# ZhangT-tech/MoCA-Video

Hardware: AMD Instinct MI355X
Metric: denoising UNet-steps/sec @16x320x512 fp16 (higher is better)
Workload: dtype f16

## Files before the change

include/moca_hip.h:

```cpp
#ifndef MOCA_HIP_H
#define MOCA_HIP_H

#include <stdint.h>

#ifdef __cplusplus
extern "C" {
#endif

#define MOCA_OK            0
#define MOCA_E_BADARG     -1
#define MOCA_E_LAUNCH     -2
#define MOCA_E_NODEVICE   -3
#define MOCA_E_GRAPH      -4

#define MOCA_A_LINEAR   0
#define MOCA_A_CONV3X3  1
#define MOCA_A_TCONV3   2

#define MOCA_EP_GEGLU   1
#define MOCA_EP_OUT_F32 2
#define MOCA_FORCE_SMALL_TILE 4
#define MOCA_EP_COLSUM 16
#define MOCA_EP_LN     32
#define MOCA_EP_GELU    8
// ... 60 lines not shown
int moca_gemm_rowsum_cols(const moca_gemm_params* p);
int moca_gemm_lnfold_ok(const moca_gemm_params* p);
int moca_gemm_tattn_ok(const moca_gemm_params* p);
int moca_gemm_wgroup_ok(const moca_gemm_params* p);
int moca_gemm_cat_ok(const moca_gemm_params* p);
#define MOCA_ROUTE_SMALL64   1
#define MOCA_ROUTE_SMALL128  2
#define MOCA_ROUTE_GLDS128   3
#define MOCA_ROUTE_GLDS160   4
#define MOCA_ROUTE_G4        5
#define MOCA_ROUTE_W80       6
#define MOCA_ROUTE_W80W      7
#define MOCA_ROUTE_SQ256     8
#define MOCA_ROUTE_G4P       9
#define MOCA_ROUTE_SQP       10
#define MOCA_ROUTE_TATTN     11
#define MOCA_ROUTE_WS        12
int moca_gemm_route(const moca_gemm_params* p);
int moca_gemm_splitk_groupnorm_ok(const moca_gemm_params* p, int32_t HW, int32_t frames_per_stat);
int moca_gemm_splitk_groupnorm_f16(const moca_gemm_params* p, void* y, const float* gamma, const float* beta, int32_t HW,
                                   int32_t frames_per_stat, float eps, int32_t silu, int32_t write_x, void* stream);
int64_t moca_gemm_splitk_ws_bytes(int32_t M, int32_t N, int32_t splits);

int moca_groupnorm_nhwc_f16(const void* x, void* y, const float* gamma, const float* beta,
                            int32_t F, int32_t HW, int32_t C, int32_t frames_per_stat,
                            float eps, int32_t silu, float* ws, void* stream);
int64_t moca_groupnorm_ws_bytes(int32_t F, int32_t HW, int32_t C);
int moca_groupnorm_colsum_f16(const void* x, void* y, const float* gamma, const float* beta, const float* colsum,
                              int32_t tile_rows, int32_t F, int32_t HW, int32_t C, int32_t frames_per_stat,
                              float eps, int32_t silu, float* ws, void* stream);

int moca_groupnorm_fold_weights_f16(const void* w, const float* bias, const float* gamma, const float* beta, const int64_t* gstat,
                                    void* wg, float* bg, int32_t n_sg, int32_t N, int32_t K, int32_t ldw, int64_t count, float eps,
                                    void* stream);

int moca_groupnorm_gstat_f16(const void* x, void* y, const float* gamma, const float* beta, const int64_t* gstat,
                             int32_t F, int32_t HW, int32_t C, int32_t frames_per_stat,
                             float eps, int32_t silu, void* stream);
int moca_concat_channels_gstat_f16(const void* a, const void* b, void* out, int32_t F, int32_t HW, int32_t C1, int32_t C2,
                                   int32_t frames_per_stat, int64_t* gstat, void* stream);
int moca_groupnorm_gstat_cat_f16(const void* a, const void* b, void* y, const float* gamma, const float* beta,
                                 const int64_t* gstat_cat, const int64_t* gstat_b, int32_t Fb, int32_t F, int32_t HW, int32_t C1,
                                 int32_t C2, int32_t frames_per_stat, float eps, int32_t silu, void* stream);
int moca_gstat_accum_f16(const void* x, int32_t F, int32_t HW, int32_t C, int32_t frames_per_stat, int32_t cpg, int32_t coff,
                         int64_t* gstat, void* stream);
int moca_memset_zero(void* ptr, int64_t bytes, void* stream);
// ... 163 lines not shown
```

moca_video_amd/lib.py:

```python
from __future__ import annotations

import ctypes as C
import os

import torch

_HERE = os.path.dirname(os.path.abspath(__file__))
LIB_PATH = os.environ.get("MOCA_HIP_LIB") or os.path.join(_HERE, "libmoca_hip.so")

MOCA_A_LINEAR, MOCA_A_CONV3X3, MOCA_A_TCONV3 = 0, 1, 2
MOCA_EP_GEGLU, MOCA_EP_OUT_F32, MOCA_FORCE_SMALL_TILE, MOCA_EP_GELU, MOCA_EP_COLSUM, MOCA_EP_LN = 1, 2, 4, 8, 16, 32
MOCA_EP_ROWSUM, MOCA_EP_LNFOLD, MOCA_EP_GSTAT, MOCA_EP_TATTN, MOCA_EP_SLABS = 64, 128, 256, 512, 1024
MOCA_TUNE_GEMM_W80, MOCA_TUNE_GEMM_G4, MOCA_TUNE_GEMM_SQ256, MOCA_TUNE_GEMM_WIDE, MOCA_TUNE_GN_SLAB, MOCA_TUNE_GEMM_G4P, MOCA_TUNE_GEMM_MF32, MOCA_TUNE_GEMM_SQP, MOCA_TUNE_SQP_WALK = 0, 1, 2, 3, 4, 5, 6, 7, 8
MOCA_TUNE_SLAB_F16 = 9
MOCA_TUNE_GEMM_WS = 10
(MOCA_ROUTE_SMALL64, MOCA_ROUTE_SMALL128, MOCA_ROUTE_GLDS128, MOCA_ROUTE_GLDS160, MOCA_ROUTE_G4, MOCA_ROUTE_W80, MOCA_ROUTE_W80W,
 MOCA_ROUTE_SQ256, MOCA_ROUTE_G4P, MOCA_ROUTE_SQP, MOCA_ROUTE_TATTN, MOCA_ROUTE_WS) = range(1, 13)

_ERR = {0: "ok", -1: "bad argument (shape/alignment contract)", -2: "HIP launch/runtime error",
        -3: "no gfx950 device", -4: "graph capture/replay failed"}


class MocaHipError(RuntimeError):
    pass
# ... 30 lines not shown
    _fields_ = [
        ("state", C.c_void_p), ("x", C.c_void_p), ("eps_c", C.c_void_p), ("eps_u", C.c_void_p), ("noise", C.c_void_p),
        ("momentum", C.c_void_p), ("queue", C.c_void_p), ("x_prev", C.c_void_p), ("pred_x0", C.c_void_p), ("coef", C.c_void_p),
        ("win_start", C.c_void_p), ("mask", C.c_void_p), ("mask_sums", C.c_void_p), ("mask_frame", C.c_void_p),
        ("enh", C.c_void_p), ("cond", C.c_void_p), ("sam_eff", C.c_void_p), ("sam_idx", C.c_void_p),
        ("cfg_scale", C.c_float), ("beta", C.c_float), ("one_minus_beta", C.c_float), ("gamma", C.c_float),
        ("one_minus_gamma", C.c_float),
        ("nW", C.c_int32), ("C", C.c_int32), ("Q", C.c_int32), ("f", C.c_int32), ("HW", C.c_int32), ("wb_from", C.c_int32),
    ]


_vp, _i32, _i64, _f32, _f64 = C.c_void_p, C.c_int32, C.c_int64, C.c_float, C.c_double
SIGNATURES = {
    "moca_gemm_f16": (C.c_int, [C.POINTER(GemmParams), _vp]),
    "moca_gemm_splitk_ws_bytes": (_i64, [_i32, _i32, _i32]),
    "moca_gemm_colsum_rows": (C.c_int, [C.POINTER(GemmParams)]),
    "moca_gemm_ln_ok": (C.c_int, [C.POINTER(GemmParams)]),
    "moca_gemm_rowsum_cols": (C.c_int, [C.POINTER(GemmParams)]),
    "moca_gemm_lnfold_ok": (C.c_int, [C.POINTER(GemmParams)]),
    "moca_gemm_tattn_ok": (C.c_int, [C.POINTER(GemmParams)]),
    "moca_gemm_cat_ok": (C.c_int, [C.POINTER(GemmParams)]),
    "moca_gemm_wgroup_ok": (C.c_int, [C.POINTER(GemmParams)]),
    "moca_gemm_route": (C.c_int, [C.POINTER(GemmParams)]),
    "moca_groupnorm_fold_weights_f16": (C.c_int, [_vp, _vp, _vp, _vp, _vp, _vp, _vp, _i32, _i32, _i32, _i32, _i64, _f32, _vp]),
    "moca_gemm_splitk_groupnorm_ok": (C.c_int, [C.POINTER(GemmParams), _i32, _i32]),
    "moca_gemm_splitk_groupnorm_f16": (C.c_int, [C.POINTER(GemmParams), _vp, _vp, _vp, _i32, _i32, _f32, _i32, _i32, _vp]),
    "moca_groupnorm_gstat_cat_f16": (C.c_int, [_vp, _vp, _vp, _vp, _vp, _vp, _vp, _i32, _i32, _i32, _i32, _i32, _i32, _f32, _i32, _vp]),
    "moca_gstat_accum_f16": (C.c_int, [_vp, _i32, _i32, _i32, _i32, _i32, _i32, _vp, _vp]),
    "moca_groupnorm_colsum_f16": (C.c_int, [_vp, _vp, _vp, _vp, _vp, _i32, _i32, _i32, _i32, _i32, _f32, _i32, _vp, _vp]),
    "moca_groupnorm_nhwc_f16": (C.c_int, [_vp, _vp, _vp, _vp, _i32, _i32, _i32, _i32, _f32, _i32, _vp, _vp]),
    "moca_groupnorm_ws_bytes": (_i64, [_i32, _i32, _i32]),
    "moca_groupnorm_gstat_f16": (C.c_int, [_vp, _vp, _vp, _vp, _vp, _i32, _i32, _i32, _i32, _f32, _i32, _vp]),
    "moca_memset_zero": (C.c_int, [_vp, _i64, _vp]),
    "moca_concat_channels_gstat_f16": (C.c_int, [_vp, _vp, _vp, _i32, _i32, _i32, _i32, _i32, _vp, _vp]),
    "moca_layernorm_f16": (C.c_int, [_vp, _vp, _vp, _vp, _i32, _i32, _f32, _vp]),
    "moca_attention_f16": (C.c_int, [_vp, _vp, _vp, _vp, _i32, _i32, _i32, _i32, _i32, _i32, _i32, _i32, _i32, _f32, _vp]),
    "moca_attention_ip_f16": (C.c_int, [_vp, _vp, _vp, _vp, _vp, _vp] + [_i32] * 12 + [_f32, _f32, _vp]),
    "moca_attention_causal_f16": (C.c_int, [_vp, _vp, _vp, _vp, _i32, _i32, _i32, _i32, _i32, _i32, _i32, _f32, _vp]),
    "moca_embed_tokens_f16": (C.c_int, [_vp, _vp, _vp, _vp, _i32, _i32, _i32, _i32, _vp]),
    "moca_attention_d80_f16": (C.c_int, [_vp, _vp, _vp, _vp, _i32, _i32, _i32, _i32, _i32, _i32, _i32, _f32, _vp]),
    "moca_clip_preprocess_patches_f16": (C.c_int, [_vp, _i32, _vp, _i32, _i32, _i32, _i32, _i32, _i32, _i32, _vp]),
    "moca_clip_assemble_tokens_f16": (C.c_int, [_vp, _i32, _vp, _vp, _vp, _i32, _i32, _i32, _vp]),
    "moca_temporal_attention_f16": (C.c_int, [_vp, _vp, _vp, _vp, _i32, _i32, _i32, _i32, _i32, _i32, _f32, _vp]),
    "moca_temporal_attention_causal_f16": (C.c_int, [_vp, _vp, _vp, _vp, _i32, _i32, _i32, _i32, _i32, _i32, _f32, _vp]),
    "moca_ncthw_to_nhwc_f16": (C.c_int, [_vp, _i32, _vp, _i32, _i32, _i32, _i32, _i32, _vp]),
    "moca_ncthw_scatter_f16": (C.c_int, [_vp, _i32, _vp, _i32, _i32, _i32, _i32, _i32, _i32, _vp]),
# ... 101 lines not shown
```

moca_video_amd/ops.py:

```python
from __future__ import annotations

import ctypes as C
import os
import torch

from . import lib as _l

_stream = None


def set_stream(handle):
    global _stream
    _stream = handle


def current_stream():
    if _stream is None:
        return torch.cuda.current_stream().cuda_stream
    return _stream


def _st():
    return C.c_void_p(current_stream())


def _round_up(x, m):
    return (x + m - 1) // m * m


class PackedWeight:
    __slots__ = ("w", "bias", "N", "K", "n_out", "geglu", "wsum", "derived")

    def __init__(self, w, bias, N, K, n_out, geglu=False):
        self.w, self.bias, self.N, self.K, self.n_out, self.geglu = w, bias, N, K, n_out, geglu
        self.wsum = None
        self.derived = False


def _finish(w2d: torch.Tensor, bias, device, n_out=None, geglu=False) -> PackedWeight:
    n, k = w2d.shape
    npad, kpad = _round_up(n, 64), _round_up(k, 64)
    w = torch.zeros(npad, kpad, dtype=torch.float16, device=device)
    w[:n, :k] = w2d.to(device=device, dtype=torch.float16)
    b = None
    if bias is not None:
        b = torch.zeros(npad, dtype=torch.float32, device=device)
        b[:n] = bias.to(device=device, dtype=torch.float32)
    return PackedWeight(w, b, npad, k, n if n_out is None else n_out, geglu)


def pack_linear(weight, bias=None, device="cuda"):
    w = weight.reshape(weight.shape[0], -1)
    return _finish(w, bias, device)


def pack_linear_cat(weights, biases=None, device="cuda"):
    w = torch.cat([x.reshape(x.shape[0], -1) for x in weights], dim=0)
    b = None
    if biases is not None:
# ... 106 lines not shown
    if tattn is not None:
        p.flags |= _l.MOCA_EP_TATTN
        p.T, p.HW, p.tattn_scale = tattn[:3]
        p.tattn_causal = 1 if len(tattn) > 3 and tattn[3] else 0
    if gstat is not None:
        p.flags |= _l.MOCA_EP_GSTAT
        p.gstat = gstat[0].data_ptr()
        p.gstat_rows = gstat[1]
        if len(gstat) > 2:
            p.gstat_cpg, p.gstat_coff = gstat[2], gstat[3]
    if lnfold is not None:
        p.flags |= _l.MOCA_EP_LNFOLD
        p.lnf_part = lnfold[0].data_ptr() if lnfold[0] is not None else None
        p.lnf_nparts = lnfold[1]
        p.ln_eps = lnfold[2]
        p.lnf_wsum = pw.wsum.data_ptr() if pw.wsum is not None else None
    if slabs:
        p.flags |= _l.MOCA_EP_SLABS
    p.splits = splits
    return p


def gemm(a, pw: PackedWeight, out, **kw):
    p = _gemm_params(a, pw, out, **kw)
    _l.check(_l.load().moca_gemm_f16(C.byref(p), _st()), "moca_gemm_f16")
    return out


def gemm_ln_ok(a, pw: PackedWeight, **kw):
    p = _gemm_params(a, pw, None, **kw)
    return bool(_l.load().moca_gemm_ln_ok(C.byref(p)))


def gemm_rowsum_cols(a, pw: PackedWeight, **kw):
    p = _gemm_params(a, pw, None, **kw)
    return int(_l.load().moca_gemm_rowsum_cols(C.byref(p)))


def gemm_lnfold_ok(a, pw: PackedWeight, **kw):
    p = _gemm_params(a, pw, None, **kw)
    return bool(_l.load().moca_gemm_lnfold_ok(C.byref(p)))


def gemm_wgroup_ok(a, pw: PackedWeight, **kw):
    p = _gemm_params(a, pw, None, **kw)
    return bool(_l.load().moca_gemm_wgroup_ok(C.byref(p)))


def gemm_route(a, pw: PackedWeight, out=None, **kw):
    p = _gemm_params(a, pw, out, **kw)
    return int(_l.load().moca_gemm_route(C.byref(p)))


def groupnorm_fold_weights(pw: PackedWeight, gamma, beta, gstat, wg, bg, *, n_sg, count, eps):
    _l.check(_l.load().moca_groupnorm_fold_weights_f16(_l.ptr(pw.w), _l.ptr(pw.bias) if pw.bias is not None else None, _l.ptr(gamma), _l.ptr(beta),
                                                       _l.ptr(gstat), _l.ptr(wg), _l.ptr(bg), n_sg, pw.N, pw.K, pw.w.stride(0), count, eps, _st()),
             "moca_groupnorm_fold_weights_f16")
    out = PackedWeight(wg, bg, pw.N, pw.K, pw.n_out)
    out.derived = True
    return out


def gemm_tattn_ok(a, pw: PackedWeight, **kw):
    p = _gemm_params(a, pw, None, **kw)
    return bool(_l.load().moca_gemm_tattn_ok(C.byref(p)))


def pack_qkv_per_head(wq, wk, wv, heads, bias=None, device="cuda"):
    C_ = wq.shape[0]
    assert C_ == heads * 64 and wk.shape[0] == C_ and wv.shape[0] == C_
    w = torch.stack([wq.reshape(heads, 64, -1), wk.reshape(heads, 64, -1), wv.reshape(heads, 64, -1)], dim=1).reshape(3 * C_, -1)
    b = None
    if bias is not None:
        b = torch.stack([bias[:C_].reshape(heads, 64), bias[C_:2 * C_].reshape(heads, 64), bias[2 * C_:].reshape(heads, 64)], dim=1).reshape(-1)
# ... 211 lines not shown
```

moca_video_amd/plan.py:

```python
from __future__ import annotations

import ctypes as C
import functools
import os
import warnings

import torch

from . import lib as _l
from . import ops
from .unet import (IMAGE_CONTEXT_MAX, TEXT_CONTEXT_LEN, _BasicTransformerBlock, _CatMap, _Downsample, _FMap, _Pool, _ResBlock,
                   _SpatialTransformer, _TemporalTransformer, _Upsample)

N_CU = 256


def gemm_splits(M, pw):
    nk = pw.w.shape[1] // 64
    tiles = 0
    if pw.N % 160 == 0 and not pw.geglu and M > 160:
        tiles = ((M + 319) // 320) * (pw.N // 160)
        if tiles < 200:
            tiles = 0
    if tiles == 0:
        if M > 128 and (pw.N % 128 == 0 or pw.N % 160 == 0):
            tm, bn = 256, (128 if pw.N % 128 == 0 else 160)
        else:
            tm, bn = 128, (128 if pw.N % 128 == 0 else 64)
        tiles = ((M + tm - 1) // tm) * (pw.N // bn)
    if tiles >= (N_CU * 3) // 4:
        return 1
    cap = N_CU // tiles
    if tiles >= 40:
        if nk <= 24:
            return 1
        if nk <= 100:
            return max(1, min(cap, 4))
    return max(1, min(cap, nk // 8))


PREFETCH_MIN_BYTES = int(float(os.environ.get("MOCA_PREFETCH_MIN_MB", "4")) * (1 << 20))
PREFETCH_HOST_FLOP = float(os.environ.get("MOCA_PREFETCH_HOST_GF", "50")) * 1e9
VIRTUAL_CAT = os.environ.get("MOCA_VCAT", "1") != "0"
SPLITK_GN = os.environ.get("MOCA_SKGN", "1") != "0"
GN_FOLD = os.environ.get("MOCA_GNFOLD", "1") != "0"
SPLITK_GN_ALL = os.environ.get("MOCA_SKGN", "1") == "2"


class _LNRef:
    __slots__ = ("x", "part", "nparts")

    def __init__(self, x, part, nparts):
        self.x, self.part, self.nparts = x, part, nparts


class _PlanBase:
    _defer_slabs = False

    def __init__(self, model, device):
        self.model = model
        self.device = device
        self.P = model._packed
        self.pool = _Pool(device)
        self.stream = torch.cuda.Stream(device=device) if torch.device(device).type == "cuda" else None
        self.steps = []
        self._pinned = set()
        self.graph = None
        self.graph_failed = False
# ... 594 lines not shown
        for layer in seq:
            if isinstance(layer, _ResBlock):
                nh = self.res_block(layer, h)
            elif isinstance(layer, _SpatialTransformer):
                nh = self.transformer(layer, h, True)
            elif isinstance(layer, _TemporalTransformer):
                nh = self.transformer(layer, h, False)
            elif isinstance(layer, _Downsample):
                nh = self.conv(h, self.P[id(layer.op)], stride=2)
            elif isinstance(layer, _Upsample):
                nh = self.upconv(h, layer.conv)
            else:
                raise TypeError(type(layer))
            if isinstance(h, _CatMap):
                self._drop_colsum(h.h)
                self._drop_colsum(h.skip)
                self._release(h.h.buf, h.skip.buf)
            else:
                self._release(h.buf)
                self._drop_colsum(h)
            h = nh
        return h

    def _embed_mlp(self, sq, rows_t):
        m, P, BT = self.model, self.P, self.BT
        te = self.pool.get(BT, m.model_channels)
        self._emit(ops.timestep_embedding, rows_t, te, n=BT, dim=m.model_channels)
        e1 = self.linear(te, BT, P[id(sq[0])])
        s1 = self.pool.get(BT, e1.shape[1])
        self._emit(ops.silu_add_rows, e1, 1, None, 1, s1, rows=BT, Cn=e1.shape[1], silu=True)
        e2 = self.linear(s1, BT, P[id(sq[2])])
        self._release(te, e1, s1)
        return e2

    def _build(self):
        m, P, B, T, H, W = self.model, self.P, self.B, self.T, self.H, self.W
        BT = self.BT
        emb = self._embed_mlp(m.time_embed, self.t_rows)
        femb = self._embed_mlp(m.fps_embedding, self.fps_rows) if m.fps_cond else None
        self.emb_silu = self.pool.get(BT, emb.shape[1])
        self._emit(ops.silu_add_rows, emb, 1, femb, 1, self.emb_silu, rows=BT, Cn=emb.shape[1], silu=True)
        self._release(emb, femb)
        self._pinned.add(self.emb_silu.data_ptr())
        self.emb_all = self.linear(self.emb_silu, BT, P["emb_all"])
        self._pinned.add(self.emb_all.data_ptr())
        self.kv_all = None
        if "ctx_kv_all" in P:
            self.kv_all = self.linear(self.ctx, self.ctx_rows, P["ctx_kv_all"])
            self._pinned.add(self.kv_all.data_ptr())
        self.kv_ip_all = None
        if self.ctx_img is not None:
            self.kv_ip_all = self.linear(self.ctx_img, self.img_rows, P["ctx_kv_ip_all"])
            self._pinned.add(self.kv_ip_all.data_ptr())

        FT = self.Bx * T
        Cpad = m.in_cpad
        if self.pieces is None:
            x8 = self.pool.get(FT * H * W, Cpad)
            self._emit(ops.ncthw_to_nhwc, self.x_in, x8, B=self.Bx, Cin=m.in_channels, T=T, HW=H * W, Cpad=Cpad)
            h = self.conv(_FMap(x8, FT, H, W, Cpad), P[id(m.input_blocks[0][0])])
            self._release(x8)
        else:
            self.x_rows = torch.zeros(FT * H * W, Cpad, dtype=torch.float16, device=self.device)
            self._emit(ops.ncthw_scatter, self.x_in, self.x_rows, B=self.Bx, k=self.kx, T=T, HW=H * W, Cpad=Cpad, c0=0)
            h = self.conv(_FMap(self.x_rows, FT, H, W, Cpad), P[id(m.input_blocks[0][0])])
        hs = []
        for i, module in enumerate(m.input_blocks):
            if i == 0:
                if m.addition_attention:
                    nh = self.transformer(m.init_attn[0], h, False)
                    self._release(h.buf)
                    self._drop_colsum(h)
                    h = nh
            else:
                h = self.run_seq(module, h)
            if self.adapter_in is not None and (i + 1) % 3 == 0:
                self._adapter_add(h, FT)
            hs.append(h)
            self._pinned.add(h.buf.data_ptr())
        h = self.run_seq(m.middle_block, h)
        if h.F != BT:
            h = _FMap(self._expand(h.buf, h.M, h.C), BT, h.H, h.W, h.C)
        for module in m.output_blocks:
            skip = hs.pop()
            if skip.F != h.F:
                self._pinned.discard(skip.buf.data_ptr())
                wide = self._expand(skip.buf, skip.M, skip.C)
                self._drop_colsum(skip)
# ... 4 lines not shown
            vc = self._virtual_cat(module, h, skip)
            if vc is not None:
                self._pinned.discard(skip.buf.data_ptr())
                h = self.run_seq(module, vc)
                continue
            cat = self.pool.get(h.M, h.C + skip.C)
            gst = None
            Cc = h.C + skip.C
            if isinstance(module[0], _ResBlock) and Cc % 32 == 0 and \
                    64 <= (Cc // 8) * max(1, 256 // (Cc // 8)) and Cc // 8 <= 1024:
                gst = (self._gstat_slot(h.F * 64), 1)
                self._emit(ops.concat_channels_gstat, h.buf, skip.buf, cat, gst[0], F=h.F, HW=h.H * h.W, C1=h.C, C2=skip.C,
                           frames_per_stat=1)
            else:
                self._emit(ops.concat_channels, h.buf, skip.buf, cat, rows=h.M, C1=h.C, C2=skip.C)
            self._pinned.discard(skip.buf.data_ptr())
            self._drop_colsum(h)
            self._drop_colsum(skip)
            self._release(h.buf, skip.buf)
            h = self.run_seq(module, _FMap(cat, h.F, h.H, h.W, Cc, gstat=gst))
        g = self.gn(h, P[id(m.out[0])], fps=1, eps=1e-5, silu=True)
        self._release(h.buf)
        self._drop_colsum(h)
        o = self.conv(_FMap(g, h.F, h.H, h.W, h.C), P[id(m.out[2])])
        self._release(g)
        self._emit(ops.nhwc_to_ncthw, o.buf, o.C, self.out, B=B, Cout=m.out_channels, T=T, HW=H * W)
        self._release(o.buf)
        self._finish_prefetch()

    def _adapter_add(self, h, FT):
        self._drop_colsum(h)
        assert h.gstat is None and h.gstat_own is None and not h.cs_used
        h.src, h.cs_rows = None, 0
        src = torch.empty(FT, h.C, h.H, h.W, dtype=torch.float32, device=self.device)
        self.adapter_in.append(src)
        self._emit(ops.nchw_add_rows, h.buf, src, F=h.F, Fsrc=FT, Cn=h.C, HW=h.H * h.W)

    def _virtual_cat(self, module, h, skip):
        if not VIRTUAL_CAT or not isinstance(module[0], _ResBlock) or isinstance(module[0].skip_connection, torch.nn.Identity):
            return None
        Cc, HW = h.C + skip.C, h.H * h.W
        if Cc % 32 or h.C % 64 or skip.C % 64 or Cc // 8 > 1024 or h.F != skip.F:
            return None
        pw = self.P[id(module[0].skip_connection)]
        if self._splits(h.M, pw) != 1 or not ops.gemm_cat_ok(h.buf, pw, M=h.M, lda=h.buf.stride(-2), splits=1, a2=(skip.buf, h.C)):
            return None
        gw = Cc // 32
# ... 107 lines not shown
```

Before: 64.85.

## Add specialized kernels for skinny linears, narrow-output and short-K 3x3 convs

```diff
diff --git a/include/moca_hip.h b/include/moca_hip.h
--- a/include/moca_hip.h
+++ b/include/moca_hip.h
@@ -106,6 +106,18 @@
                                    int32_t frames_per_stat, float eps, int32_t silu, int32_t write_x, void* stream);
 int64_t moca_gemm_splitk_ws_bytes(int32_t M, int32_t N, int32_t splits);
 
+int moca_linear_skinny_ok(int32_t M, int32_t N, int32_t K, int32_t lda, int32_t ldw, int32_t ldo);
+int moca_linear_skinny_f16(const void* a, const void* w, const float* bias, void* out, int32_t M, int32_t N, int32_t K,
+                           int32_t lda, int32_t ldw, int32_t ldo, void* stream);
+int moca_conv3x3_narrow_ok(int32_t F, int32_t H, int32_t W, int32_t C, int32_t n_out, int32_t ldw, int32_t ldo);
+int moca_conv3x3_narrow_f16(const void* a, const void* w, const float* bias, void* out, int32_t F, int32_t H, int32_t W,
+                            int32_t C, int32_t n_out, int32_t ldw, int32_t ldo, void* stream);
+int moca_conv3x3_shortk_ok(int32_t F, int32_t H, int32_t W, int32_t Cpad, int32_t N, int32_t ldw, int32_t ldo,
+                           int32_t gstat_rows, int32_t gstat_cpg, int32_t gstat_coff);
+int moca_conv3x3_shortk_f16(const void* a, const void* w, const float* bias, void* out, int64_t* gstat, int32_t F, int32_t H,
+                            int32_t W, int32_t Cpad, int32_t N, int32_t ldw, int32_t ldo, int32_t gstat_rows, int32_t gstat_cpg,
+                            int32_t gstat_coff, void* stream);
+
 int moca_groupnorm_nhwc_f16(const void* x, void* y, const float* gamma, const float* beta,
                             int32_t F, int32_t HW, int32_t C, int32_t frames_per_stat,
                             float eps, int32_t silu, float* ws, void* stream);
diff --git a/moca_video_amd/csrc/small_shapes.hip b/moca_video_amd/csrc/small_shapes.hip
--- /dev/null
+++ b/moca_video_amd/csrc/small_shapes.hip
@@ -0,0 +1,462 @@
+#include "common.h"
+
+namespace {
+
+typedef unsigned u32x4 __attribute__((ext_vector_type(4)));
+[[maybe_unused]] constexpr unsigned SS_OOB = 0x80000000u;
+
+__device__ __forceinline__ __amdgpu_buffer_rsrc_t ss_rsrc(const void* p, int64_t bytes) {
+    return __builtin_amdgcn_make_buffer_rsrc(const_cast<void*>(p), 0, (int)bytes, 0x00020000);
+}
+__device__ __forceinline__ half8v ss_ld16(__amdgpu_buffer_rsrc_t r, unsigned off) {
+    return __builtin_bit_cast(half8v, __builtin_amdgcn_raw_buffer_load_b128(r, (int)off, 0, 0));
+}
+
+int ss_cus() {
+    static int cached = 0;
+    if (!cached) {
+        int dev = 0;
+        hipDeviceProp_t prop;
+        if (hipGetDevice(&dev) == hipSuccess && hipGetDeviceProperties(&prop, dev) == hipSuccess && prop.multiProcessorCount > 0)
+            cached = prop.multiProcessorCount;
+        else
+            cached = 256;
+    }
+    return cached;
+}
+
+template <bool KSPLIT>
+__global__ __launch_bounds__(KSPLIT ? 256 : 512) void skinny_linear_kernel(const half_t* __restrict__ a, const half_t* __restrict__ w,
+                                                                           const float* __restrict__ bias, half_t* __restrict__ out,
+                                                                           int M, int N, int K, int lda, int ldw, int ldo) {
+#if defined(__HIP_DEVICE_COMPILE__)
+    extern __shared__ __attribute__((aligned(16))) char smem[];
+    constexpr int NW = KSPLIT ? 4 : 8, NT = NW * 64;
+    const int tid = threadIdx.x, lane = tid & 63, fr = lane & 15, fq = lane >> 4;
+    const int wave = __builtin_amdgcn_readfirstlane(tid >> 6);
+    const int U = K >> 6, nrb = M > 16 ? 2 : 1;
+    const int ct = KSPLIT ? (int)blockIdx.x : (int)blockIdx.x * NW + wave;
+    const bool live = ct < (N >> 4);
+    int u0 = 0, u1 = U;
+    if constexpr (KSPLIT) {
+        const int upw = (U + NW - 1) / NW;
+        u0 = min(U, wave * upw);
+        u1 = min(U, u0 + upw);
+    }
+    const __amdgpu_buffer_rsrc_t rsrc_w = ss_rsrc(w, (int64_t)N * ldw * 2);
+    const __amdgpu_buffer_rsrc_t rsrc_a = ss_rsrc(a, ((int64_t)(M - 1) * lda + K) * 2);
+    const unsigned wrow = live ? (unsigned)(((ct * 16 + fr) * ldw + 16 * fq) * 2) : SS_OOB;
+    half8v w0[10], w1[10];
+    auto load_w = [&](half8v (&buf)[10], int ub) {
+#pragma unroll
+        for (int i = 0; i < 5; ++i) {
+            const int u = ub + i;
+            const unsigned off = u < u1 ? wrow + (unsigned)u * 128u : SS_OOB;
+            buf[2 * i] = ss_ld16(rsrc_w, off);
+            buf[2 * i + 1] = ss_ld16(rsrc_w, off + 16u);
+        }
+    };
+    load_w(w0, u0);
+
+    const int cpr = K >> 3, total = nrb * 16 * cpr;
+    const int spare = nrb * 16 * K * 2 + (KSPLIT ? NW * 2 * 1024 : 0) + lane * 16;
+    constexpr int AU = 10;
+    for (int base = tid; base < total; base += AU * NT) {
+        half8v v[AU];
+#pragma unroll
+        for (int j = 0; j < AU; ++j) {
+            const int idx = base + j * NT, row = idx / cpr, c = idx - row * cpr;
+            v[j] = ss_ld16(rsrc_a, idx < total && row < M ? (unsigned)((row * lda + c * 8) * 2) : SS_OOB);
+        }
+#pragma unroll
+        for (int j = 0; j < AU; ++j) {
+            const int idx = base + j * NT, row = idx / cpr, c = idx - row * cpr;
+            const int frag = (row >> 4) * 2 * U + 2 * (c >> 3) + (c & 1), l = ((c >> 1) & 3) * 16 + (row & 15);
+            *reinterpret_cast<half8v*>(smem + (idx < total ? (frag * 64 + l) * 16 : spare)) = v[j];
+        }
+    }
+    __syncthreads();
+
+    f32x4 acc0 = {0.f, 0.f, 0.f, 0.f}, acc1 = {0.f, 0.f, 0.f, 0.f};
+    const char* const a_rd = smem + lane * 16;
+    auto compute = [&](const half8v (&buf)[10], int ub) {
+#pragma unroll
+        for (int i = 0; i < 5; ++i) {
+            const int u = ub + i;
+            if (u < u1) {
+#pragma unroll
+                for (int h = 0; h < 2; ++h) {
+                    const half8v a0 = *reinterpret_cast<const half8v*>(a_rd + (2 * u + h) * 1024);
+                    acc0 = __builtin_amdgcn_mfma_f32_16x16x32_f16(buf[2 * i + h], a0, acc0, 0, 0, 0);
+                    if (nrb == 2) {
+                        const half8v a1 = *reinterpret_cast<const half8v*>(a_rd + (2 * U + 2 * u + h) * 1024);
+                        acc1 = __builtin_amdgcn_mfma_f32_16x16x32_f16(buf[2 * i + h], a1, acc1, 0, 0, 0);
+                    }
+                }
+            }
+        }
+    };
+    for (int ub = u0; ub < u1; ub += 10) {
+        load_w(w1, ub + 5);
+        compute(w0, ub);
+        load_w(w0, ub + 10);
+        compute(w1, ub + 5);
+    }
+
+    if constexpr (KSPLIT) {
+        float* const ex = reinterpret_cast<float*>(smem + nrb * 16 * K * 2);
+        *reinterpret_cast<f32x4*>(ex + ((wave * 2 + 0) * 64 + lane) * 4) = acc0;
+        *reinterpret_cast<f32x4*>(ex + ((wave * 2 + 1) * 64 + lane) * 4) = acc1;
+        __syncthreads();
+        if (wave != 0) return;
+        acc0 = *reinterpret_cast<const f32x4*>(ex + lane * 4);
+        acc1 = *reinterpret_cast<const f32x4*>(ex + (64 + lane) * 4);
+#pragma unroll
+        for (int wv = 1; wv < NW; ++wv) {
+            acc0 += *reinterpret_cast<const f32x4*>(ex + ((wv * 2 + 0) * 64 + lane) * 4);
+            acc1 += *reinterpret_cast<const f32x4*>(ex + ((wv * 2 + 1) * 64 + lane) * 4);
+        }
+    }
+    if (!live) return;
+    const int n = ct * 16 + 4 * fq;
+    f32x4 b = {0.f, 0.f, 0.f, 0.f};
+    if (bias) b = *reinterpret_cast<const f32x4*>(bias + n);
+    if (fr < M) {
+        const half4v o = {(half_t)(acc0[0] + b[0]), (half_t)(acc0[1] + b[1]), (half_t)(acc0[2] + b[2]), (half_t)(acc0[3] + b[3])};
+        *reinterpret_cast<half4v*>(out + (int64_t)fr * ldo + n) = o;
+    }
+    if (16 + fr < M) {
+        const half4v o = {(half_t)(acc1[0] + b[0]), (half_t)(acc1[1] + b[1]), (half_t)(acc1[2] + b[2]), (half_t)(acc1[3] + b[3])};
+        *reinterpret_cast<half4v*>(out + (int64_t)(16 + fr) * ldo + n) = o;
+    }
+#endif
+}
+
+[[maybe_unused]] constexpr int NC_G = 5, NC_NL = 9;
+__global__ __launch_bounds__(512) void conv3x3_narrow_kernel(const half_t* __restrict__ a, const half_t* __restrict__ w,
+                                                             const float* __restrict__ bias, half_t* __restrict__ out, int M, int H,
+                                                             int W, int C, int ldw, int ldo) {
+#if defined(__HIP_DEVICE_COMPILE__)
+    extern __shared__ __attribute__((aligned(16))) char smem[];
+    const int tid = threadIdx.x, lane = tid & 63, fr = lane & 15, fq = lane >> 4;
+    const int wave = __builtin_amdgcn_readfirstlane(tid >> 6);
+    const int cs = C >> 5, KS = 9 * cs, ncp = cs >> 1;
+    const int npix = NC_G * 64 + 2 * W + 2;
+    const int zslot = KS * 1024, spare = zslot + 128 + lane * 16, abase = zslot + 128 + 1024;
+    if (tid < 8) *reinterpret_cast<half8v*>(smem + zslot + tid * 16) = half8v{0, 0, 0, 0, 0, 0, 0, 0};
+    const __amdgpu_buffer_rsrc_t rsrc_w = ss_rsrc(w, (int64_t)16 * ldw * 2);
+    for (int base = tid; base < KS * 64; base += 6 * 512) {
+        half8v v[6];
+#pragma unroll
+        for (int j = 0; j < 6; ++j) {
+            const int idx = base + j * 512, sk = idx >> 6, l = idx & 63;
+            v[j] = ss_ld16(rsrc_w, idx < KS * 64 ? (unsigned)(((l & 15) * ldw + 32 * sk + 8 * (l >> 4)) * 2) : SS_OOB);
+        }
+#pragma unroll
+        for (int j = 0; j < 6; ++j) {
+            const int idx = base + j * 512;
+            *reinterpret_cast<half8v*>(smem + (idx < KS * 64 ? idx * 16 : spare)) = v[j];
+        }
+    }
+    const __amdgpu_buffer_rsrc_t rsrc_a = ss_rsrc(a, (int64_t)M * C * 2);
+    f32x4 b = {0.f, 0.f, 0.f, 0.f};
+    if (bias) b = *reinterpret_cast<const f32x4*>(bias + 4 * fq);
+    const int n_tiles = (M + 63) >> 6, n_groups = (n_tiles + NC_G - 1) / NC_G, HW = H * W;
+    const int my_groups = n_groups > (int)blockIdx.x ? (n_groups - 1 - (int)blockIdx.x) / (int)gridDim.x + 1 : 0;
+    const int n_it = my_groups * ncp;
+    half8v R[NC_NL];
+    auto load_chunk = [&](int it) {
+        const int gi = it / ncp, cp = it - gi * ncp;
+        const int q0 = ((int)blockIdx.x + gi * (int)gridDim.x) * NC_G * 64 - W - 1;
+#pragma unroll
+        for (int j = 0; j < NC_NL; ++j) {
+            const int idx = tid + 512 * j, pl = idx >> 3, c = idx & 7, q = q0 + pl;
+            R[j] = ss_ld16(rsrc_a, pl < npix && q >= 0 && q < M ? (unsigned)((q * C + cp * 64 + c * 8) * 2) : SS_OOB);
+        }
+    };
+    if (n_it > 0) load_chunk(0);
+    unsigned addr[4][9];
+    f32x4 acc[4];
+    int tile = 0;
+    bool has = false;
+    const char* const w_rd = smem + lane * 16;
+    for (int it = 0; it < n_it; ++it) {
+        const int gi = it / ncp, cp = it - gi * ncp;
+        if (cp == 0) {
+            tile = ((int)blockIdx.x + gi * (int)gridDim.x) * NC_G + wave;
+            has = wave < NC_G && tile < n_tiles;
+#pragma unroll
+            for (int t = 0; t < 4; ++t) {
+                acc[t] = f32x4{0.f, 0.f, 0.f, 0.f};
+                const int p = tile * 64 + 16 * t + fr, pp = p < M ? p : 0;
+                const int r = pp % HW, y = r / W, x = r - y * W;
+#pragma unroll
+                for (int tap = 0; tap < 9; ++tap) {
+                    const int dy = tap / 3 - 1, dx = tap % 3 - 1;
+                    const bool ok = p < M && y + dy >= 0 && y + dy < H && x + dx >= 0 && x + dx < W;
+                    const int pl = wave * 64 + 16 * t + fr + W + 1 + dy * W + dx;
+                    addr[t][tap] = ok ? (unsigned)(abase + pl * 128 + ((fq ^ ((pl >> 1) & 7)) << 4)) : (unsigned)(zslot + fq * 16);
+                }
+            }
+        }
+        __syncthreads();
+#pragma unroll
+        for (int j = 0; j < NC_NL; ++j) {
+            const int idx = tid + 512 * j, pl = idx >> 3, c = idx & 7;
+            *reinterpret_cast<half8v*>(smem + (pl < npix ? abase + pl * 128 + ((c ^ ((pl >> 1) & 7)) << 4) : spare)) = R[j];
+        }
+        __syncthreads();
+        load_chunk(min(it + 1, n_it - 1));
+        if (has) {
+#pragma unroll
+            for (int tap = 0; tap < 9; ++tap)
+#pragma unroll
+                for (int h = 0; h < 2; ++h) {
+                    const half8v wf = *reinterpret_cast<const half8v*>(w_rd + (tap * cs + 2 * cp + h) * 1024);
+#pragma unroll
+                    for (int t = 0; t < 4; ++t) {
+                        const half8v av = *reinterpret_cast<const half8v*>(smem + (addr[t][tap] ^ (unsigned)(h * 64)));
+                        acc[t] = __builtin_amdgcn_mfma_f32_16x16x32_f16(wf, av, acc[t], 0, 0, 0);
+                    }
+                }
+            if (cp == ncp - 1) {
+#pragma unroll
+                for (int t = 0; t < 4; ++t) {
+                    const int p = tile * 64 + 16 * t + fr;
+                    if (p < M) {
+                        const half4v o = {(half_t)(acc[t][0] + b[0]), (half_t)(acc[t][1] + b[1]), (half_t)(acc[t][2] + b[2]),
+                                          (half_t)(acc[t][3] + b[3])};
+                        *reinterpret_cast<half4v*>(out + (int64_t)p * ldo + 4 * fq) = o;
+                    }
+                }
+            }
+        }
+    }
+#endif
+}
+
+[[maybe_unused]] constexpr int SK_ROWS = 160, SK_PITCH = 328;
+template <int CPAD>
+__global__ __launch_bounds__(640) void conv3x3_shortk_kernel(const half_t* __restrict__ a, const half_t* __restrict__ w,
+                                                             const float* __restrict__ bias, half_t* __restrict__ out,
+                                                             int64_t* __restrict__ gstat, int M, int H, int W, int N, int ldw, int ldo,
+                                                             int gstat_rows, int cpg, int coff) {
+#if defined(__HIP_DEVICE_COMPILE__)
+    extern __shared__ __attribute__((aligned(16))) char smem[];
+    constexpr int KS = CPAD == 8 ? 3 : 5;
+    const int tid = threadIdx.x, lane = tid & 63, fr = lane & 15, fq = lane >> 4;
+    const int wave = __builtin_amdgcn_readfirstlane(tid >> 6);
+    const int rg = wave % 5, ch = wave / 5;
+    const int m0 = (int)blockIdx.x * SK_ROWS, n0 = (int)blockIdx.y * 320;
+    const int ncols = min(320, N - n0), rows = min(SK_ROWS, M - m0);
+    const int HW = H * W;
+
+    const __amdgpu_buffer_rsrc_t rsrc_a = ss_rsrc(a, (int64_t)M * CPAD * 2);
+    half8v af[2][KS];
+#pragma unroll
+    for (int rt = 0; rt < 2; ++rt) {
+        const int m = m0 + rg * 32 + rt * 16 + fr, mm = m < M ? m : 0;
+        const int r = mm % HW, y = r / W, x = r - y * W;
+#pragma unroll
+        for (int s = 0; s < KS; ++s) {
+            const int tap = CPAD == 8 ? 4 * s + fq : 2 * s + (fq >> 1), c0 = CPAD == 8 ? 0 : 8 * (fq & 1);
+            const int ky = tap / 3, kx = tap - 3 * ky, yy = y + ky - 1, xx = x + kx - 1;
+            const bool ok = m < M && tap < 9 && yy >= 0 && yy < H && xx >= 0 && xx < W;
+            af[rt][s] = ss_ld16(rsrc_a, ok ? (unsigned)(((mm + (ky - 1) * W + (kx - 1)) * CPAD + c0) * 2) : SS_OOB);
+        }
+    }
+    const __amdgpu_buffer_rsrc_t rsrc_w = ss_rsrc(w, (int64_t)N * ldw * 2);
+    {
+        half8v wv[2 * KS];
+#pragma unroll
+        for (int i = 0; i < 2 * KS; ++i) {
+            const int idx = tid + 640 * i, j = idx / (KS * 64), rem = idx - j * KS * 64, s = rem >> 6, l = rem & 63;
+            const int col = 16 * j + (l & 15);
+            wv[i] = ss_ld16(rsrc_w, col < ncols ? (unsigned)(((n0 + col) * ldw + 32 * s + 8 * (l >> 4)) * 2) : SS_OOB);
+        }
+#pragma unroll
+        for (int i = 0; i < 2 * KS; ++i) *reinterpret_cast<half8v*>(smem + (tid + 640 * i) * 16) = wv[i];
+    }
+    __syncthreads();
+    f32x4 acc[2][10];
+#pragma unroll
+    for (int j = 0; j < 10; ++j) { acc[0][j] = f32x4{0.f, 0.f, 0.f, 0.f}; acc[1][j] = f32x4{0.f, 0.f, 0.f, 0.f}; }
+    const bool cols_live = ch * 160 < ncols;
+    if (cols_live) {
+        const char* const w_rd = smem + (ch * 10 * KS * 64 + lane) * 16;
+#pragma unroll
+        for (int s = 0; s < KS; ++s)
+#pragma unroll
+            for (int j = 0; j < 10; ++j) {
+                const half8v wf = *reinterpret_cast<const half8v*>(w_rd + (j * KS + s) * 1024);
+                acc[0][j] = __builtin_amdgcn_mfma_f32_16x16x32_f16(wf, af[0][s], acc[0][j], 0, 0, 0);
+                acc[1][j] = __builtin_amdgcn_mfma_f32_16x16x32_f16(wf, af[1][s], acc[1][j], 0, 0, 0);
+            }
+    }
+    __syncthreads();
+    half_t* const stage = reinterpret_cast<half_t*>(smem);
+    if (cols_live) {
+#pragma unroll
+        for (int j = 0; j < 10; ++j) {
+            const int col = ch * 160 + 16 * j + 4 * fq;
+            f32x4 b = {0.f, 0.f, 0.f, 0.f};
+            if (bias) b = *reinterpret_cast<const f32x4*>(bias + n0 + col);
+#pragma unroll
+            for (int rt = 0; rt < 2; ++rt) {
+                const half4v o = {(half_t)(acc[rt][j][0] + b[0]), (half_t)(acc[rt][j][1] + b[1]), (half_t)(acc[rt][j][2] + b[2]),
+                                  (half_t)(acc[rt][j][3] + b[3])};
+                *reinterpret_cast<half4v*>(stage + (rg * 32 + rt * 16 + fr) * SK_PITCH + col) = o;
+            }
+        }
+    }
+    __syncthreads();
+    const int cpr = ncols >> 3;
+#pragma unroll 5
+    for (int idx = tid; idx < rows * cpr; idx += 640) {
+        const int row = idx / cpr, c = idx - row * cpr;
+        *reinterpret_cast<half8v*>(out + (int64_t)(m0 + row) * ldo + n0 + 8 * c) = *reinterpret_cast<const half8v*>(stage + row * SK_PITCH + 8 * c);
+    }
+    if (!gstat) return;
+    float* const part = reinterpret_cast<float*>(smem + SK_ROWS * SK_PITCH * 2);
+    const int g0 = (coff + n0) / cpg, g1 = (coff + n0 + ncols - 1) / cpg;
+    const int c = tid % 320, sub = tid / 320;
+    for (int sg = m0 / gstat_rows; sg <= (m0 + rows - 1) / gstat_rows; ++sg) {
+        const int r0 = max(sg * gstat_rows, m0) - m0, r1 = min((sg + 1) * gstat_rows, m0 + rows) - m0;
+        float s = 0.f, q = 0.f;
+        if (c < ncols)
+#pragma unroll 8
+            for (int r = r0 + sub; r < r1; r += 2) {
+                const float v = (float)stage[r * SK_PITCH + c];
+                s += v;
+                q += v * v;
+            }
+        part[(sub * 320 + c) * 2] = s;
+        part[(sub * 320 + c) * 2 + 1] = q;
+        __syncthreads();
+        if (tid < 2 * (g1 - g0 + 1)) {
+            const int g = g0 + (tid >> 1), comp = tid & 1;
+            const int c0 = max(g * cpg - coff, n0) - n0, c1 = min((g + 1) * cpg - coff, n0 + ncols) - n0;
+            float t = 0.f;
+            for (int cc = c0; cc < c1; ++cc) t += part[cc * 2 + comp] + part[(320 + cc) * 2 + comp];
+            moca_gstat_add(gstat + ((int64_t)sg * 32 + g) * 2 + comp, comp, t);
+        }
+        __syncthreads();
+    }
+#endif
+}
+
+bool ss_aligned16(const void* p) { return (reinterpret_cast<uintptr_t>(p) & 15) == 0; }
+
+template <typename Kern>
+int ss_allow_lds(Kern kern, bool* done, size_t lds) {
+    if (lds > 64 * 1024 && !*done) {
+        if (hipFuncSetAttribute(reinterpret_cast<const void*>(kern), hipFuncAttributeMaxDynamicSharedMemorySize, 160 * 1024) != hipSuccess)
+            return MOCA_E_LAUNCH;
+        *done = true;
+    }
+    return MOCA_OK;
+}
+
+}
+
+extern "C" int moca_linear_skinny_ok(int32_t M, int32_t N, int32_t K, int32_t lda, int32_t ldw, int32_t ldo) {
+    if (M < 1 || M > 32 || N < 16 || N % 16 || K < 64 || K > 1280 || K % 64) return 0;
+    if (lda < K || lda % 8 || ldw < K || ldw % 8 || ldo < N || ldo % 4) return 0;
+    if ((int64_t)N * ldw * 2 >= (1ll << 31)) return 0;
+    return 1;
+}
+
+extern "C" int moca_linear_skinny_f16(const void* a, const void* w, const float* bias, void* out, int32_t M, int32_t N, int32_t K,
+                                      int32_t lda, int32_t ldw, int32_t ldo, void* stream) {
+    if (!a || !w || !out || !moca_linear_skinny_ok(M, N, K, lda, ldw, ldo)) return MOCA_E_BADARG;
+    if (!ss_aligned16(a) || !ss_aligned16(w) || !ss_aligned16(bias) || (reinterpret_cast<uintptr_t>(out) & 7)) return MOCA_E_BADARG;
+    const int tiles = N / 16;
+    const size_t a_bytes = (size_t)(M > 16 ? 32 : 16) * K * 2;
+    const half_t* ah = reinterpret_cast<const half_t*>(a);
+    const half_t* wh = reinterpret_cast<const half_t*>(w);
+    half_t* oh = reinterpret_cast<half_t*>(out);
+    if (tiles >= 512) {
+        static bool attr = false;
+        const size_t lds = a_bytes + 1024;
+        if (ss_allow_lds(&skinny_linear_kernel<false>, &attr, lds)) return MOCA_E_LAUNCH;
+        hipLaunchKernelGGL(skinny_linear_kernel<false>, dim3((tiles + 7) / 8), dim3(512), lds, moca_stream(stream), ah, wh, bias, oh, M, N, K,
+                           lda, ldw, ldo);
+    } else {
+        static bool attr = false;
+        const size_t lds = a_bytes + 4 * 2 * 64 * 16 + 1024;
+        if (ss_allow_lds(&skinny_linear_kernel<true>, &attr, lds)) return MOCA_E_LAUNCH;
+        hipLaunchKernelGGL(skinny_linear_kernel<true>, dim3(tiles), dim3(256), lds, moca_stream(stream), ah, wh, bias, oh, M, N, K, lda, ldw, ldo);
+    }
+    MOCA_CHECK_LAUNCH();
+    return MOCA_OK;
+}
+
+static size_t narrow_lds_bytes(int C, int W) { return (size_t)9 * (C / 32) * 1024 + 128 + 1024 + (size_t)(NC_G * 64 + 2 * W + 2) * 128; }
+
+extern "C" int moca_conv3x3_narrow_ok(int32_t F, int32_t H, int32_t W, int32_t C, int32_t n_out, int32_t ldw, int32_t ldo) {
+    if (F < 1 || H < 1 || W < 1 || C < 64 || C > 320 || C % 64 || n_out < 1 || n_out > 16) return 0;
+    if (ldw < 9 * C || ldw % 8 || ldo < 16 || ldo % 4) return 0;
+    if ((int64_t)F * H * W * C * 2 >= (1ll << 31)) return 0;
+    if ((NC_G * 64 + 2 * (int64_t)W + 2) * 8 > NC_NL * 512 || narrow_lds_bytes(C, W) > 160 * 1024) return 0;
+    return 1;
+}
+
+extern "C" int moca_conv3x3_narrow_f16(const void* a, const void* w, const float* bias, void* out, int32_t F, int32_t H, int32_t W,
+                                       int32_t C, int32_t n_out, int32_t ldw, int32_t ldo, void* stream) {
+    if (!a || !w || !out || !moca_conv3x3_narrow_ok(F, H, W, C, n_out, ldw, ldo)) return MOCA_E_BADARG;
+    if (!ss_aligned16(a) || !ss_aligned16(w) || !ss_aligned16(bias) || (reinterpret_cast<uintptr_t>(out) & 7)) return MOCA_E_BADARG;
+    const int M = F * H * W, n_groups = ((M + 63) / 64 + NC_G - 1) / NC_G;
+    const size_t lds = narrow_lds_bytes(C, W);
+    static bool attr = false;
+    if (ss_allow_lds(&conv3x3_narrow_kernel, &attr, lds)) return MOCA_E_LAUNCH;
+    hipLaunchKernelGGL(conv3x3_narrow_kernel, dim3(n_groups < ss_cus() ? n_groups : ss_cus()), dim3(512), lds, moca_stream(stream),
+                       reinterpret_cast<const half_t*>(a), reinterpret_cast<const half_t*>(w), bias, reinterpret_cast<half_t*>(out), M, H, W, C,
+                       ldw, ldo);
+    MOCA_CHECK_LAUNCH();
+    return MOCA_OK;
+}
+
+extern "C" int moca_conv3x3_shortk_ok(int32_t F, int32_t H, int32_t W, int32_t Cpad, int32_t N, int32_t ldw, int32_t ldo,
+                                      int32_t gstat_rows, int32_t gstat_cpg, int32_t gstat_coff) {
+    if (F < 1 || H < 1 || W < 1 || (Cpad != 8 && Cpad != 16) || N < 160 || N % 160) return 0;
+    const int KS = Cpad == 8 ? 3 : 5;
+    if (ldw < 32 * KS || ldw % 8 || ldo < N || ldo % 8) return 0;
+    const int64_t M = (int64_t)F * H * W;
+    if (M * Cpad * 2 >= (1ll << 31) || (int64_t)N * ldw * 2 >= (1ll << 31) || (M + SK_ROWS - 1) / SK_ROWS > 0x7fffffff) return 0;
+    if (gstat_rows < 0 || gstat_cpg < 0 || gstat_coff < 0) return 0;
+    if (gstat_rows > 0) {
+        if (M % gstat_rows) return 0;
+        if (gstat_cpg > 0 ? (gstat_coff + N - 1) / gstat_cpg >= 32 : (N % 32 != 0 || gstat_coff != 0)) return 0;
+    } else if (gstat_cpg || gstat_coff) {
+        return 0;
+    }
+    return 1;
+}
+
+extern "C" int moca_conv3x3_shortk_f16(const void* a, const void* w, const float* bias, void* out, int64_t* gstat, int32_t F, int32_t H,
+                                       int32_t W, int32_t Cpad, int32_t N, int32_t ldw, int32_t ldo, int32_t gstat_rows, int32_t gstat_cpg,
+                                       int32_t gstat_coff, void* stream) {
+    if (!a || !w || !out || !moca_conv3x3_shortk_ok(F, H, W, Cpad, N, ldw, ldo, gstat_rows, gstat_cpg, gstat_coff)) return MOCA_E_BADARG;
+    if ((gstat != nullptr) != (gstat_rows > 0)) return MOCA_E_BADARG;
+    if (!ss_aligned16(a) || !ss_aligned16(w) || !ss_aligned16(bias) || !ss_aligned16(out)) return MOCA_E_BADARG;
+    const int M = F * H * W;
+    const int cpg = gstat_cpg > 0 ? gstat_cpg : N / 32;
+    const dim3 grid((M + SK_ROWS - 1) / SK_ROWS, (N + 319) / 320);
+    const size_t lds = (size_t)SK_ROWS * SK_PITCH * 2 + 2 * 320 * 2 * sizeof(float);
+    const half_t* ah = reinterpret_cast<const half_t*>(a);
+    const half_t* wh = reinterpret_cast<const half_t*>(w);
+    half_t* oh = reinterpret_cast<half_t*>(out);
+    if (Cpad == 8) {
+        static bool attr = false;
+        if (ss_allow_lds(&conv3x3_shortk_kernel<8>, &attr, lds)) return MOCA_E_LAUNCH;
+        hipLaunchKernelGGL(conv3x3_shortk_kernel<8>, grid, dim3(640), lds, moca_stream(stream), ah, wh, bias, oh, gstat, M, H, W, N, ldw, ldo,
+                           gstat_rows, cpg, gstat_coff);
+    } else {
+        static bool attr = false;
+        if (ss_allow_lds(&conv3x3_shortk_kernel<16>, &attr, lds)) return MOCA_E_LAUNCH;
+        hipLaunchKernelGGL(conv3x3_shortk_kernel<16>, grid, dim3(640), lds, moca_stream(stream), ah, wh, bias, oh, gstat, M, H, W, N, ldw, ldo,
+                           gstat_rows, cpg, gstat_coff);
+    }
+    MOCA_CHECK_LAUNCH();
+    return MOCA_OK;
+}
diff --git a/moca_video_amd/lib.py b/moca_video_amd/lib.py
--- a/moca_video_amd/lib.py
+++ b/moca_video_amd/lib.py
@@ -76,6 +76,12 @@
     "moca_gemm_cat_ok": (C.c_int, [C.POINTER(GemmParams)]),
     "moca_gemm_wgroup_ok": (C.c_int, [C.POINTER(GemmParams)]),
     "moca_gemm_route": (C.c_int, [C.POINTER(GemmParams)]),
+    "moca_linear_skinny_ok": (C.c_int, [_i32] * 6),
+    "moca_linear_skinny_f16": (C.c_int, [_vp, _vp, _vp, _vp] + [_i32] * 6 + [_vp]),
+    "moca_conv3x3_narrow_ok": (C.c_int, [_i32] * 7),
+    "moca_conv3x3_narrow_f16": (C.c_int, [_vp, _vp, _vp, _vp] + [_i32] * 7 + [_vp]),
+    "moca_conv3x3_shortk_ok": (C.c_int, [_i32] * 10),
+    "moca_conv3x3_shortk_f16": (C.c_int, [_vp, _vp, _vp, _vp, _vp] + [_i32] * 10 + [_vp]),
     "moca_groupnorm_fold_weights_f16": (C.c_int, [_vp, _vp, _vp, _vp, _vp, _vp, _vp, _i32, _i32, _i32, _i32, _i64, _f32, _vp]),
     "moca_gemm_splitk_groupnorm_ok": (C.c_int, [C.POINTER(GemmParams), _i32, _i32]),
     "moca_gemm_splitk_groupnorm_f16": (C.c_int, [C.POINTER(GemmParams), _vp, _vp, _vp, _i32, _i32, _f32, _i32, _i32, _vp]),
diff --git a/moca_video_amd/ops.py b/moca_video_amd/ops.py
--- a/moca_video_amd/ops.py
+++ b/moca_video_amd/ops.py
@@ -1,6 +1,7 @@
 from __future__ import annotations
 
 import ctypes as C
+import functools
 import os
 import torch
 
@@ -29,12 +30,13 @@
 
 
 class PackedWeight:
-    __slots__ = ("w", "bias", "N", "K", "n_out", "geglu", "wsum", "derived")
+    __slots__ = ("w", "bias", "N", "K", "n_out", "geglu", "wsum", "derived", "small")
 
     def __init__(self, w, bias, N, K, n_out, geglu=False):
         self.w, self.bias, self.N, self.K, self.n_out, self.geglu = w, bias, N, K, n_out, geglu
         self.wsum = None
         self.derived = False
+        self.small = False
 
 
 def _finish(w2d: torch.Tensor, bias, device, n_out=None, geglu=False) -> PackedWeight:
@@ -187,9 +189,42 @@
 
 
 def gemm(a, pw: PackedWeight, out, **kw):
+    if pw.small:
+        fn = small_entry(a, pw, out, **kw)
+        if fn is not None:
+            return fn()
     p = _gemm_params(a, pw, out, **kw)
     _l.check(_l.load().moca_gemm_f16(C.byref(p), _st()), "moca_gemm_f16")
     return out
+
+
+def small_entry(a, pw: PackedWeight, out, **kw):
+    if not pw.small or pw.geglu or out is None:
+        return None
+    kw = {k: v for k, v in kw.items() if v is not None}
+    M, mode, gstat = kw.pop("M"), kw.pop("mode", _l.MOCA_A_LINEAR), kw.pop("gstat", None)
+    conv, lda = kw.pop("conv", None), kw.pop("lda", None)
+    kw.pop("splits", None), kw.pop("splitk_ws", None)
+    kw.pop("prefetch", None)
+    if kw.pop("rowadd_div", 1) != 1 or kw.pop("up_phase", 0) or kw:
+        return None
+    if mode == _l.MOCA_A_LINEAR:
+        if gstat is None and linear_skinny_ok(a, pw, M=M, lda=lda) and out.stride(-2) >= pw.N:
+            return functools.partial(linear_skinny, a, pw, out, M=M, lda=lda)
+        return None
+    if mode != _l.MOCA_A_CONV3X3 or conv is None or lda is not None:
+        return None
+    Cn, H, W = conv[0], conv[1], conv[2]
+    if conv[5] != 1 or conv[6] or (H, W) != (conv[3], conv[4]) or (len(conv) > 7 and conv[7]) or M % (H * W):
+        return None
+    F = M // (H * W)
+    if Cn <= 16:
+        if pw.n_out == pw.N and conv3x3_shortk_ok(pw, F=F, H=H, W=W, Cpad=Cn, ldo=out.stride(-2), gstat=gstat):
+            return functools.partial(conv3x3_shortk, a, pw, out, F=F, H=H, W=W, Cpad=Cn, gstat=gstat)
+        return None
+    if gstat is None and pw.n_out <= 16 and conv3x3_narrow_ok(pw, F=F, H=H, W=W, Cn=Cn, n_out=pw.n_out, ldo=out.stride(-2)):
+        return functools.partial(conv3x3_narrow, a, pw, out, F=F, H=H, W=W, Cn=Cn, n_out=pw.n_out)
+    return None
 
 
 def gemm_ln_ok(a, pw: PackedWeight, **kw):
@@ -215,6 +250,52 @@
 def gemm_route(a, pw: PackedWeight, out=None, **kw):
     p = _gemm_params(a, pw, out, **kw)
     return int(_l.load().moca_gemm_route(C.byref(p)))
+
+
+def linear_skinny_ok(a, pw: PackedWeight, *, M, lda=None):
+    if pw.geglu or pw.wsum is not None:
+        return False
+    lda = lda if lda is not None else a.stride(-2)
+    return bool(_l.load().moca_linear_skinny_ok(M, pw.N, pw.K, lda, pw.w.stride(0), pw.N))
+
+
+def linear_skinny(a, pw: PackedWeight, out, *, M, lda=None):
+    lda = lda if lda is not None else a.stride(-2)
+    _l.check(_l.load().moca_linear_skinny_f16(_l.ptr(a), _l.ptr(pw.w), _l.ptr(pw.bias), _l.ptr(out), M, pw.N, pw.K, lda, pw.w.stride(0),
+                                              out.stride(-2), _st()), "moca_linear_skinny_f16")
+    return out
+
+
+def conv3x3_narrow_ok(pw: PackedWeight, *, F, H, W, Cn, n_out, ldo):
+    if pw.geglu or pw.K != 9 * Cn or pw.w.shape[0] < 16:
+        return False
+    return bool(_l.load().moca_conv3x3_narrow_ok(F, H, W, Cn, n_out, pw.w.stride(0), ldo))
+
+
+def conv3x3_narrow(a, pw: PackedWeight, out, *, F, H, W, Cn, n_out):
+    _l.check(_l.load().moca_conv3x3_narrow_f16(_l.ptr(a), _l.ptr(pw.w), _l.ptr(pw.bias), _l.ptr(out), F, H, W, Cn, n_out, pw.w.stride(0),
+                                               out.stride(-2), _st()), "moca_conv3x3_narrow_f16")
+    return out
+
+
+def _shortk_gstat(gstat):
+    if gstat is None:
+        return None, 0, 0, 0
+    return gstat[0], gstat[1], (gstat[2] if len(gstat) > 2 else 0), (gstat[3] if len(gstat) > 2 else 0)
+
+
+def conv3x3_shortk_ok(pw: PackedWeight, *, F, H, W, Cpad, ldo, gstat=None):
+    if pw.geglu or pw.K != 9 * Cpad:
+        return False
+    _, rows, cpg, coff = _shortk_gstat(gstat)
+    return bool(_l.load().moca_conv3x3_shortk_ok(F, H, W, Cpad, pw.n_out, pw.w.stride(0), ldo, rows, cpg, coff))
+
+
+def conv3x3_shortk(a, pw: PackedWeight, out, *, F, H, W, Cpad, gstat=None):
+    slot, rows, cpg, coff = _shortk_gstat(gstat)
+    _l.check(_l.load().moca_conv3x3_shortk_f16(_l.ptr(a), _l.ptr(pw.w), _l.ptr(pw.bias), _l.ptr(out), _l.ptr(slot), F, H, W, Cpad, pw.n_out,
+                                               pw.w.stride(0), out.stride(-2), rows, cpg, coff, _st()), "moca_conv3x3_shortk_f16")
+    return out
 
 
 def groupnorm_fold_weights(pw: PackedWeight, gamma, beta, gstat, wg, bg, *, n_sg, count, eps):
diff --git a/moca_video_amd/plan.py b/moca_video_amd/plan.py
--- a/moca_video_amd/plan.py
+++ b/moca_video_amd/plan.py
@@ -44,6 +44,7 @@
 VIRTUAL_CAT = os.environ.get("MOCA_VCAT", "1") != "0"
 SPLITK_GN = os.environ.get("MOCA_SKGN", "1") != "0"
 GN_FOLD = os.environ.get("MOCA_GNFOLD", "1") != "0"
+SMALL_SHAPES = os.environ.get("MOCA_SMALL", "1") != "0"
 SPLITK_GN_ALL = os.environ.get("MOCA_SKGN", "1") == "2"
 
 
@@ -684,14 +685,18 @@
             h = nh
         return h
 
+    def _small(self, pw):
+        pw.small = SMALL_SHAPES
+        return pw
+
     def _embed_mlp(self, sq, rows_t):
         m, P, BT = self.model, self.P, self.BT
         te = self.pool.get(BT, m.model_channels)
         self._emit(ops.timestep_embedding, rows_t, te, n=BT, dim=m.model_channels)
-        e1 = self.linear(te, BT, P[id(sq[0])])
+        e1 = self.linear(te, BT, self._small(P[id(sq[0])]))
         s1 = self.pool.get(BT, e1.shape[1])
         self._emit(ops.silu_add_rows, e1, 1, None, 1, s1, rows=BT, Cn=e1.shape[1], silu=True)
-        e2 = self.linear(s1, BT, P[id(sq[2])])
+        e2 = self.linear(s1, BT, self._small(P[id(sq[2])]))
         self._release(te, e1, s1)
         return e2
 
@@ -704,7 +709,7 @@
         self._emit(ops.silu_add_rows, emb, 1, femb, 1, self.emb_silu, rows=BT, Cn=emb.shape[1], silu=True)
         self._release(emb, femb)
         self._pinned.add(self.emb_silu.data_ptr())
-        self.emb_all = self.linear(self.emb_silu, BT, P["emb_all"])
+        self.emb_all = self.linear(self.emb_silu, BT, self._small(P["emb_all"]))
         self._pinned.add(self.emb_all.data_ptr())
         self.kv_all = None
         if "ctx_kv_all" in P:
@@ -720,12 +725,12 @@
         if self.pieces is None:
             x8 = self.pool.get(FT * H * W, Cpad)
             self._emit(ops.ncthw_to_nhwc, self.x_in, x8, B=self.Bx, Cin=m.in_channels, T=T, HW=H * W, Cpad=Cpad)
-            h = self.conv(_FMap(x8, FT, H, W, Cpad), P[id(m.input_blocks[0][0])])
+            h = self.conv(_FMap(x8, FT, H, W, Cpad), self._small(P[id(m.input_blocks[0][0])]))
             self._release(x8)
         else:
             self.x_rows = torch.zeros(FT * H * W, Cpad, dtype=torch.float16, device=self.device)
             self._emit(ops.ncthw_scatter, self.x_in, self.x_rows, B=self.Bx, k=self.kx, T=T, HW=H * W, Cpad=Cpad, c0=0)
-            h = self.conv(_FMap(self.x_rows, FT, H, W, Cpad), P[id(m.input_blocks[0][0])])
+            h = self.conv(_FMap(self.x_rows, FT, H, W, Cpad), self._small(P[id(m.input_blocks[0][0])]))
         hs = []
         for i, module in enumerate(m.input_blocks):
             if i == 0:
@@ -776,7 +781,7 @@
         g = self.gn(h, P[id(m.out[0])], fps=1, eps=1e-5, silu=True)
         self._release(h.buf)
         self._drop_colsum(h)
-        o = self.conv(_FMap(g, h.F, h.H, h.W, h.C), P[id(m.out[2])])
+        o = self.conv(_FMap(g, h.F, h.H, h.W, h.C), self._small(P[id(m.out[2])]))
         self._release(g)
         self._emit(ops.nhwc_to_ncthw, o.buf, o.C, self.out, B=B, Cout=m.out_channels, T=T, HW=H * W)
         self._release(o.buf)
```

Measured after the change: 65.03 (median of 6 runs). About the same (+0.3%).
